# earth-insights/ZoomEarth

Hardware: AMD Instinct MI355X
Metric: questions/sec end-to-end, ZoomEarth-3B on 5000px tiles (higher is better)
Workload: dtype bf16

## Files before the change

### include/zoomearth.h

```cpp
#ifndef ZOOMEARTH_H
#define ZOOMEARTH_H

#include <stddef.h>
#include <stdint.h>

#ifdef __cplusplus
extern "C" {
#endif

typedef struct ze_engine ze_engine;

typedef enum {
    ZE_OK = 0,
    ZE_ERR_INVALID = -1,
    ZE_ERR_HIP = -2,
    ZE_ERR_NOMEM = -3,
    ZE_ERR_NOTFOUND = -4,
    ZE_ERR_MISMATCH = -5
} ze_status;

typedef enum { ZE_F32 = 0, ZE_F16 = 1, ZE_BF16 = 2 } ze_dtype;

#define ZE_MAX_FULLATT 16
#define ZE_MAX_EOS 4
// ... 170 lines not shown
                      float* out_rows, int32_t* out_stop, void* stream);

#define ZE_MAX_GRAMMARS 16
#define ZE_MAX_GRAMMAR_STATES 2048
#define ZE_MAX_GRAMMAR_CLASSES 4096
int ze_grammar_create(ze_engine* e, const uint16_t* token_class, int n_classes, const int16_t* trans, int n_states,
                      const uint8_t* accepting, int* out_grammar, void* stream);
int ze_grammar_destroy(ze_engine* e, int grammar);
int ze_seq_set_grammar(ze_engine* e, int seq, int grammar, int state, void* stream);
int ze_chain_grammar_state(ze_engine* e, int seq, int* state, int* violated, void* stream);
int ze_op_grammar_mask(ze_engine* e, int grammar, const float* logits, int rows, int vocab, int ld, const int32_t* states, float* out,
                       void* stream);
int ze_op_grammar_advance(ze_engine* e, int grammar, const int32_t* states, const int32_t* tokens, int rows, int32_t* out_states,
                          void* stream);

int ze_weights_quantize_fp8(ze_engine* e, void* stream);
int ze_set_fp8_activations(ze_engine* e, int on);
int ze_op_quantize_fp8(ze_engine* e, void* w_bf16, int rows, int cols, void* q_out, void* scale_out, void* stream);
int ze_op_linear_mx(ze_engine* e, const void* a8, const void* sa, const void* w8, const void* sw, const void* bias, void* c,
                    int M, int N, int K, int swiglu, void* stream);

#define ZE_WEIGHTS_BF16 0
#define ZE_WEIGHTS_FP8 1
#define ZE_WEIGHTS_MXFP4 2
int ze_weights_quantize_mxfp4(ze_engine* e, void* stream);
int ze_op_quantize_mxfp4(ze_engine* e, void* w_bf16, int rows, int cols, void* q_out, void* scale_out, void* stream);
int ze_op_gemv4(ze_engine* e, int epi, const void* q4, const void* scale_e8m0, const void* x_bf16, const void* norm_w, float eps,
                const void* bias_bf16, int N, int K, void* out_bf16, float* out_f32, const uint8_t* seen, float penalty,
                int32_t* out_token, int seq, int layer, const void* embed, int token, void* embed_out, void* stream);
int ze_weight_format(ze_engine* e);

int ze_op_linear(ze_engine* e, const void* a_bf16, const void* w_bf16, const void* bias_bf16, void* c_bf16, int M,
                 int N, int K, int act, void* stream);
int ze_op_rmsnorm(ze_engine* e, const void* x_bf16, const void* weight_bf16, void* y_bf16, int rows, int cols,
                  float eps, void* stream);
int ze_op_token_logprob(ze_engine* e, const void* logits_bf16, int rows, int vocab, int ld, const int32_t* targets,
                        float* out, void* stream);
int ze_op_score_detail(ze_engine* e, const void* logits_bf16, int rows, int vocab, int ld, const int32_t* targets, int top_n,
                       float* out_logprob, float* out_entropy, int32_t* out_rank, int32_t* out_top_ids, float* out_top_logprobs,
                       void* stream);
int ze_op_attention(ze_engine* e, const void* q, const void* k, const void* v, void* o, int T, int heads,
                    int kv_heads, int D, const int32_t* cu_seqlens, int n_seg, int causal, void* stream);

int ze_op_window_gather(ze_engine* e, const float* pixel_values, const int32_t* grid_thw, int n_images, void* out_bf16, void* stream);
int ze_op_window_scatter(ze_engine* e, const void* x_bf16, int cols, const int32_t* grid_thw, int n_images, void* out_bf16,
                         void* stream);
int ze_op_vision_rope(ze_engine* e, void* qkv_bf16, const int32_t* grid_thw, int n_images, int window_order, void* stream);
int ze_op_embed_scatter(ze_engine* e, const int32_t* input_ids, int len, const void* image_embeds, int n_image_rows, void* out_bf16,
                        void* stream);
int ze_op_mrope_kv(ze_engine* e, int seq, int layer, void* qkv_bf16, int T, const int32_t* position_ids, int past, void* stream);
int ze_op_rope_kv_decode(ze_engine* e, const int32_t* seqs, int n, int layer, void* qkv_bf16, void* stream);
int ze_op_kv_read(ze_engine* e, int seq, int layer, int start, int n, void* out_k, void* out_v, void* stream);

int ze_seq_set_speculation(ze_engine* e, int seq, int k, int min_ngram, int max_ngram, const int32_t* prompt_ids, int n_prompt, void* stream);
int ze_chain_spec_stats(ze_engine* e, int seq, int* steps, int* drafted, int* accepted, void* stream);
int ze_op_spec_draft(ze_engine* e, const int32_t* hist_ids, const int32_t* hist_lens, int rows, int ld, int k, int min_ngram,
                     int max_ngram, int32_t* out_draft, int32_t* out_len, void* stream);
int ze_op_spec_accept(ze_engine* e, const float* logits, int n_chains, int vocab, int ld, int k, const int32_t* draft,
                      const int32_t* draft_len, uint8_t* seen, const float* repetition_penalty, const int32_t* room, int ignore_eos,
                      int32_t* out_tokens, int32_t* out_count, int32_t* out_finished, void* stream);
int ze_op_decode_rows(ze_engine* e, int seq, const int32_t* tokens, int r, float* out_logits, void* stream);
int ze_op_attn_decode(ze_engine* e, const int32_t* seqs, int n, int layer, const void* qkv_bf16, void* out_bf16, void* stream);
int ze_op_attn_decode_single(ze_engine* e, int seq, int layer, const void* qkv_bf16, void* out_bf16, void* stream);
int ze_op_gemv(ze_engine* e, int epi, const void* w_bf16, const void* w8, const void* scale8, const void* x_bf16, const void* norm_w,
               float eps, const void* bias_bf16, int act8, int N, int K, void* out_bf16, float* out_f32, const uint8_t* seen,
               float penalty, int32_t* out_token, int seq, int layer, const void* embed, int token, void* embed_out, void* stream);
// ... 20 lines not shown
```

### zoomearth_amd/_lib.py

```python
from __future__ import annotations

import ctypes as C
import os
import subprocess

_HERE = os.path.dirname(os.path.abspath(__file__))
LIB_PATH = os.environ.get("ZE_LIB_PATH") or os.path.join(_HERE, "libzoomearth_hip.so")
CSRC = os.path.join(_HERE, "csrc")

ZE_F32, ZE_F16, ZE_BF16 = 0, 1, 2
ZE_MAX_FULLATT, ZE_MAX_EOS = 16, 4


class ZeConfig(C.Structure):
    _fields_ = [
        ("vit_depth", C.c_int32), ("vit_hidden", C.c_int32), ("vit_heads", C.c_int32),
        ("vit_intermediate", C.c_int32), ("vit_out_hidden", C.c_int32),
        ("patch_size", C.c_int32), ("temporal_patch_size", C.c_int32), ("spatial_merge_size", C.c_int32),
        ("window_size", C.c_int32), ("in_channels", C.c_int32),
        ("n_fullatt", C.c_int32), ("fullatt_block_indexes", C.c_int32 * ZE_MAX_FULLATT),
        ("hidden", C.c_int32), ("layers", C.c_int32), ("heads", C.c_int32), ("kv_heads", C.c_int32),
        ("intermediate", C.c_int32), ("vocab", C.c_int32),
        ("rms_eps", C.c_float), ("rope_theta", C.c_float), ("mrope_section", C.c_int32 * 3),
        ("tie_word_embeddings", C.c_int32),
# ... 130 lines not shown
                                         C.POINTER(C.c_float), _P, _P]),
    "ze_op_sample_rows": (C.c_int, [_P, _P, C.c_int, C.c_int, C.c_int, _P, C.POINTER(C.c_float), C.POINTER(C.c_float),
                                    C.POINTER(C.c_uint64), C.POINTER(C.c_int32), C.POINTER(C.c_int32), C.POINTER(C.c_int32),
                                    C.POINTER(C.c_float), C.POINTER(C.c_float), _P, _P]),
    "ze_seq_set_logprobs": (C.c_int, [_P, C.c_int, C.c_int, _P]),
    "ze_chain_logprobs": (C.c_int, [_P, C.c_int, C.POINTER(C.c_float), C.POINTER(C.c_int32), C.POINTER(C.c_float), C.c_int,
                                    C.POINTER(C.c_int), C.POINTER(C.c_int), _P]),
    "ze_chain_logprobs_batch": (C.c_int, [_P, C.POINTER(C.c_int32), C.c_int, C.POINTER(C.c_float), C.POINTER(C.c_int32),
                                          C.POINTER(C.c_float), C.c_int, C.c_int, C.POINTER(C.c_int32), _P]),
    "ze_op_token_logprobs": (C.c_int, [_P, _P, C.c_int, C.c_int, C.c_int, _P, C.c_int, _P, _P, _P, _P]),
    "ze_seq_set_logit_adjust": (C.c_int, [_P, C.c_int, C.c_float, C.c_float, C.c_int, C.POINTER(C.c_int32), C.POINTER(C.c_float),
                                          C.c_int, _P]),
    "ze_op_logit_adjust": (C.c_int, [_P, _P, C.c_int, C.c_int, C.c_int, _P, _P, _P, _P, _P, _P, _P, _P, _P]),
    "ze_seq_set_token_rules": (C.c_int, [_P, C.c_int, C.c_int, C.POINTER(C.c_int32), C.c_int, C.POINTER(C.c_int32), C.c_int,
                                         C.POINTER(C.c_int32), C.c_int, _P]),
    "ze_op_token_rules": (C.c_int, [_P, _P, C.c_int, C.c_int, C.c_int, _P, _P, _P, _P, _P, _P, _P, _P, _P, _P, _P, _P]),
    "ze_grammar_create": (C.c_int, [_P, C.POINTER(C.c_uint16), C.c_int, C.POINTER(C.c_int16), C.c_int, C.POINTER(C.c_uint8),
                                    C.POINTER(C.c_int), _P]),
    "ze_grammar_destroy": (C.c_int, [_P, C.c_int]),
    "ze_seq_set_grammar": (C.c_int, [_P, C.c_int, C.c_int, C.c_int, _P]),
    "ze_chain_grammar_state": (C.c_int, [_P, C.c_int, C.POINTER(C.c_int), C.POINTER(C.c_int), _P]),
    "ze_op_grammar_mask": (C.c_int, [_P, C.c_int, _P, C.c_int, C.c_int, C.c_int, _P, _P, _P]),
    "ze_op_grammar_advance": (C.c_int, [_P, C.c_int, _P, _P, C.c_int, _P, _P]),
    "ze_weights_quantize_fp8": (C.c_int, [_P, _P]),
    "ze_set_fp8_activations": (C.c_int, [_P, C.c_int]),
    "ze_op_quantize_fp8": (C.c_int, [_P, _P, C.c_int, C.c_int, _P, _P, _P]),
    "ze_weights_quantize_mxfp4": (C.c_int, [_P, _P]),
    "ze_op_quantize_mxfp4": (C.c_int, [_P, _P, C.c_int, C.c_int, _P, _P, _P]),
    "ze_op_gemv4": (C.c_int, [_P, C.c_int, _P, _P, _P, _P, C.c_float, _P, C.c_int, C.c_int, _P, _P, _P, C.c_float,
                              C.POINTER(C.c_int32), C.c_int, C.c_int, _P, C.c_int, _P, _P]),
    "ze_weight_format": (C.c_int, [_P]),
    "ze_op_linear_mx": (C.c_int, [_P, _P, _P, _P, _P, _P, _P, C.c_int, C.c_int, C.c_int, C.c_int, _P]),
    "ze_op_linear": (C.c_int, [_P, _P, _P, _P, _P, C.c_int, C.c_int, C.c_int, C.c_int, _P]),
    "ze_op_rmsnorm": (C.c_int, [_P, _P, _P, _P, C.c_int, C.c_int, C.c_float, _P]),
    "ze_op_attention": (C.c_int, [_P, _P, _P, _P, _P, C.c_int, C.c_int, C.c_int, C.c_int, C.POINTER(C.c_int32),
                                  C.c_int, C.c_int, _P]),
    "ze_op_window_gather": (C.c_int, [_P, _P, C.POINTER(C.c_int32), C.c_int, _P, _P]),
    "ze_op_window_scatter": (C.c_int, [_P, _P, C.c_int, C.POINTER(C.c_int32), C.c_int, _P, _P]),
    "ze_op_vision_rope": (C.c_int, [_P, _P, C.POINTER(C.c_int32), C.c_int, C.c_int, _P]),
    "ze_op_embed_scatter": (C.c_int, [_P, C.POINTER(C.c_int32), C.c_int, _P, C.c_int, _P, _P]),
    "ze_op_mrope_kv": (C.c_int, [_P, C.c_int, C.c_int, _P, C.c_int, C.POINTER(C.c_int32), C.c_int, _P]),
    "ze_op_rope_kv_decode": (C.c_int, [_P, C.POINTER(C.c_int32), C.c_int, C.c_int, _P, _P]),
    "ze_op_attn_decode": (C.c_int, [_P, C.POINTER(C.c_int32), C.c_int, C.c_int, _P, _P, _P]),
    "ze_op_attn_decode_single": (C.c_int, [_P, C.c_int, C.c_int, _P, _P, _P]),
    "ze_op_kv_read": (C.c_int, [_P, C.c_int, C.c_int, C.c_int, C.c_int, _P, _P, _P]),
    "ze_seq_set_speculation": (C.c_int, [_P, C.c_int, C.c_int, C.c_int, C.c_int, C.POINTER(C.c_int32), C.c_int, _P]),
    "ze_chain_spec_stats": (C.c_int, [_P, C.c_int, C.POINTER(C.c_int), C.POINTER(C.c_int), C.POINTER(C.c_int), _P]),
    "ze_op_spec_draft": (C.c_int, [_P, _P, _P, C.c_int, C.c_int, C.c_int, C.c_int, C.c_int, _P, _P, _P]),
    "ze_op_spec_accept": (C.c_int, [_P, _P, C.c_int, C.c_int, C.c_int, C.c_int, _P, _P, _P, _P, _P, C.c_int, _P, _P, _P, _P]),
    "ze_op_decode_rows": (C.c_int, [_P, C.c_int, C.POINTER(C.c_int32), C.c_int, _P, _P]),
    "ze_op_gemv": (C.c_int, [_P, C.c_int, _P, _P, _P, _P, _P, C.c_float, _P, C.c_int, C.c_int, C.c_int, _P, _P, _P, C.c_float,
                             C.POINTER(C.c_int32), C.c_int, C.c_int, _P, C.c_int, _P, _P]),
    "ze_op_logits_rows": (C.c_int, [_P, _P, _P, C.c_float, _P, _P, C.c_int, C.c_int, C.c_int, _P]),
    "ze_op_numeric_helpers": (C.c_int, [_P, _P, _P, _P, _P, C.c_int, _P]),
    "ze_profile_decode_kernel": (C.c_int, [_P, C.c_int, C.c_int, C.POINTER(C.c_float), C.POINTER(C.c_double), _P]),
    "ze_profile_batch_kernel": (C.c_int, [_P, C.c_int, C.c_int, C.c_int, C.POINTER(C.c_float), C.POINTER(C.c_double), _P]),
    "ze_profile_prefill_kernel": (C.c_int, [_P, C.c_int, C.c_int, C.c_int, C.POINTER(C.c_float), C.POINTER(C.c_double), _P]),
    "ze_profile_prefill_layer": (C.c_int, [_P, C.c_int, C.c_int, C.POINTER(C.c_float), C.POINTER(C.c_double), _P]),
    "ze_phase_timers": (C.c_int, [_P, C.c_int, C.c_int, C.POINTER(C.c_float)]),
    "ze_tune": (C.c_int, [C.c_int, C.c_int]),
}
EXPORTS = tuple(_SIGS)


def lib():
    global _lib
# ... 25 lines not shown
```

### zoomearth_amd/csrc/ze_forward.hip

```cpp
#include <math.h>
#include <cmath>
#include <string.h>

#include <algorithm>

#include "ze_engine.h"

extern int ze_gemv_knobs[24];

static int frontend_acquire(ze_engine* e) {
    if (e->fe_in_flight) {
        ZE_HIP(hipEventSynchronize(e->fe_done));
        e->fe_in_flight = false;
    }
    return ZE_OK;
}
static int frontend_release(ze_engine* e, hipStream_t s) {
    if (!e->fe_done) ZE_HIP(hipEventCreateWithFlags(&e->fe_done, hipEventDisableTiming));
    ZE_HIP(hipEventRecord(e->fe_done, s));
    e->fe_in_flight = true;
    return ZE_OK;
}
static int stage_acquire(ze_engine* e, hipEvent_t& ev) {
    if (ev) ZE_HIP(hipEventSynchronize(ev));
// ... 2122 lines not shown
        if (act == 5)
            ze_launch_gemm_oneshot(ZE_EPI_NONE, xf, wf, (const bf16_t*)bias, nullptr, 0, (bf16_t*)cmat, N, M, N, K, s);
        else
            ze_launch_gemm_frag(ZE_EPI_NONE, xf, wf, (const bf16_t*)bias, nullptr, 0, (bf16_t*)cmat, N, M, N, K, s);
        hipStreamSynchronize(s);
        hipFree(wf);
    } else if (act == 4) {
        if (N % 32) return ze_fail(e, ZE_ERR_INVALID, "SwiGLU: N = 2 * width with width % 16 == 0");
        ze_launch_gemm(ZE_EPI_SWIGLU, (const bf16_t*)a, K, (const bf16_t*)w, K, (const bf16_t*)bias, nullptr, 0,
                       (bf16_t*)cmat, N / 2, nullptr, M, N, K, s, e->prefill_ws());
    } else if (act == 6 || act == 7) {
        if (act == 7 && N % 32) return ze_fail(e, ZE_ERR_INVALID, "SwiGLU: N = 2 * width with width % 16 == 0");
        ze_launch_gemm_wide(act == 7 ? ZE_EPI_SWIGLU : ZE_EPI_NONE, (const bf16_t*)a, K, (const bf16_t*)w, K, (const bf16_t*)bias,
                            nullptr, 0, (bf16_t*)cmat, act == 7 ? N / 2 : N, M, N, K, e->gemm_ws(), s);
    } else if (act == 10) {
        ze_launch_gemm_wide(ZE_EPI_F32, (const bf16_t*)a, K, (const bf16_t*)w, K, nullptr, nullptr, 0, (bf16_t*)cmat, N, M, N, K,
                            e->gemm_ws(), s);
    } else if (act == 8 || act == 9) {
        if (act == 9 && N % 32) return ze_fail(e, ZE_ERR_INVALID, "SwiGLU: N = 2 * width with width % 16 == 0");
        if (K % 64 || K < 64) return ze_fail(e, ZE_ERR_INVALID, "eight-phase kernel: K a multiple of 64");
        ze_launch_gemm_p8(act == 9 ? ZE_EPI_SWIGLU : ZE_EPI_NONE, (const bf16_t*)a, K, (const bf16_t*)w, K, (const bf16_t*)bias, nullptr, 0,
                          (bf16_t*)cmat, act == 9 ? N / 2 : N, nullptr, M, N, K, s, e->prefill_ws());
    } else if (act == 2) {
        ze_launch_gemm_stream(ZE_EPI_NONE, (const bf16_t*)a, K, (const bf16_t*)w, K, (const bf16_t*)bias, nullptr, 0,
                              (bf16_t*)cmat, N, M, N, K, e->gemm_ws(), s);
    } else {
        ze_launch_gemm(act ? ZE_EPI_GELU : ZE_EPI_NONE, (const bf16_t*)a, K, (const bf16_t*)w, K, (const bf16_t*)bias,
                       nullptr, 0, (bf16_t*)cmat, N, nullptr, M, N, K, s, e->prefill_ws());
    }
    ZE_KCHECK();
    return ZE_OK;
}

extern "C" int ze_op_token_logprob(ze_engine* e, const void* logits, int rows, int vocab, int ld, const int32_t* targets,
                                   float* out, void* stream) {
    if (!logits || !targets || !out || rows < 0 || vocab <= 0 || ld < vocab || ld % 8)
        return ze_fail(e, ZE_ERR_INVALID, "bad token_logprob arguments");
    hipSetDevice(e->device);
    ze_launch_token_logprob((const bf16_t*)logits, ld, vocab, targets, out, rows, (hipStream_t)stream);
    ZE_KCHECK();
    return ZE_OK;
}

extern "C" int ze_op_score_detail(ze_engine* e, const void* logits, int rows, int vocab, int ld, const int32_t* targets, int top_n,
                                  float* out_logprob, float* out_entropy, int32_t* out_rank, int32_t* out_top_ids,
                                  float* out_top_logprobs, void* stream) {
    if (!e || !logits || !targets || !out_logprob || rows < 0 || vocab <= 0 || ld < vocab || ld % 8)
        return ze_fail(e, ZE_ERR_INVALID, "bad score_detail arguments");
    if (top_n < 0 || top_n > ZE_MAX_TOP_LOGPROBS) return ze_fail(e, ZE_ERR_INVALID, "top_n must be in [0, 20]");
    if (!out_top_ids != !out_top_logprobs || (out_top_ids && top_n < 1))
        return ze_fail(e, ZE_ERR_INVALID, "the top arrays are both null, or both set with top_n >= 1");
    hipSetDevice(e->device);
    ze_launch_score_detail((const bf16_t*)logits, ld, vocab, targets, out_top_ids ? top_n : 0, out_logprob, out_entropy, out_rank,
                           out_top_ids, out_top_logprobs, rows, (hipStream_t)stream);
    ZE_KCHECK();
    return ZE_OK;
}

extern "C" int ze_op_rmsnorm(ze_engine* e, const void* x, const void* weight, void* y, int rows, int cols, float eps,
                             void* stream) {
    if (!e || !x || !weight || !y) return ze_fail(e, ZE_ERR_INVALID, "null argument");
    if (cols % 8) return ze_fail(e, ZE_ERR_INVALID, "cols must be a multiple of 8");
    hipSetDevice(e->device);
    ze_launch_rmsnorm((const bf16_t*)x, cols, (const bf16_t*)weight, (bf16_t*)y, cols, rows, cols, eps,
                      (hipStream_t)stream);
    ZE_KCHECK();
// ... 508 lines not shown
```

### zoomearth_amd/csrc/ze_gemm.hip

```cpp
#include <algorithm>
#include <type_traits>

#include "ze_kernels.h"

typedef __attribute__((ext_vector_type(8))) __bf16 bf16x8;
typedef __attribute__((ext_vector_type(4))) float f32x4;
typedef __attribute__((ext_vector_type(4))) unsigned int u32x4;

#define GEMM_BK 64

extern int ze_live_engines;
extern int ze_gemv_knobs[24];

__device__ __forceinline__ float gelu_erf(float x) { return 0.5f * x * (1.0f + erff(x * 0.70710678118654752440f)); }

template <int BM, int BN, int EPI, int WM = 2, int WN = 2, bool LDS_EPI = false>
__device__ __forceinline__ void gemm_finish(f32x4 (&acc)[BM / (16 * WM)][BN / (16 * WN)], uint8_t* smem, const bf16_t* __restrict__ bias,
                                            const bf16_t* __restrict__ R, int ldr, bf16_t* __restrict__ C, int ldc,
                                            const int* __restrict__ c_rows, int M, int N, int ksplit, int ks, int bid,
                                            int nwg, int bm0, int bn0, float* __restrict__ slab,
                                            unsigned* __restrict__ tickets) {
    constexpr int TM = BM / (16 * WM), TN = BN / (16 * WN), NT = 64 * WM * WN;
    const int tid = threadIdx.x, lane = tid & 63, wid = tid >> 6;
    const int wm0 = (wid / WN) * (BM / WM), wn0 = (wid % WN) * (BN / WN);
// ... 643 lines not shown
            for (int i = 0; i < TM; ++i) {
#pragma unroll
                for (int j = 0; j < TN; ++j)
                    acc[i][j] = __builtin_amdgcn_mfma_f32_16x16x32_bf16(fa[i], fb[j], acc[i][j], 0, 0, 0);
                if (SPREAD && more) {
                    const int r = kk * TM + i;
#pragma unroll
                    for (int pc = 0; pc < LPW; ++pc)
                        if ((STAGES == 2 ? min(pc, 2 * TM - 1) : pc * (2 * TM) / LPW) == r) {
                            if (pc < LPA)
                                ring_issue_one(A, lda, bm0, M - 1, k_next, img_next, wid + pc * (NT / 64), lane);
                            else
                                ring_issue_one(W, ldw, bn0, N - 1, k_next, img_next + BM * 128,
                                               wid + (pc - LPA) * (NT / 64), lane);
                        }
                }
            }
        }
    }
    __syncthreads();
    gemm_finish<BM, BN, EPI, WM, WN, WIDE_EPI>(acc, smem, bias, R, ldr, C, ldc, c_rows, M, N, ksplit, ks, bid, nwg, bm0, bn0, slab, tickets);
}


template <int EPI>
__device__ __forceinline__ void p8_finish_wide(f32x4 (&acc)[8][4], uint8_t* scratch, const bf16_t* __restrict__ bias,
                                               const bf16_t* __restrict__ R, int ldr, bf16_t* __restrict__ C, int ldc,
                                               const int* __restrict__ c_rows, int M, int N, int row_base, int col_base, int lane) {
    constexpr bool SW = EPI == ZE_EPI_SWIGLU, F32 = EPI == ZE_EPI_F32;
    constexpr int EB = F32 ? 4 : 2;
    constexpr int OW = SW ? 32 : 64;
    constexpr int ROWB = OW * EB;
    constexpr int PPR = ROWB / 16;
    constexpr int CR = 4096 / ROWB > 32 ? 32 : 4096 / ROWB;
    constexpr int TI = CR / 16;
    const int fr = lane & 15, fq = lane >> 4;
    float b[4];
#pragma unroll
    for (int j = 0; j < 4; ++j) {
        const int ncol = col_base + j * 16 + fr;
        b[j] = (bias && ncol < N) ? bf16_to_f32(bias[ncol]) : 0.f;
    }
    const int ocol_base = SW ? col_base / 2 : col_base, on = SW ? N / 2 : N;
#pragma unroll
    for (int c = 0; c < 128 / CR; ++c) {
#pragma unroll
        for (int ii = 0; ii < TI; ++ii) {
            const int i = TI * c + ii;
#pragma unroll
            for (int j = 0; j < 4; j += (SW ? 2 : 1)) {
#pragma unroll
                for (int r = 0; r < 4; ++r) {
                    const int lrow = ii * 16 + fq * 4 + r;
                    const int swz = (lrow & (PPR - 1)) << 4;
                    float v;
                    int col;
                    if (SW) {
                        const float g = bf16_round(acc[i][j][r] + b[j]);
                        const float u = bf16_round(acc[i][j + 1][r] + b[j + 1]);
                        v = bf16_round(silu_f(g)) * u;
                        col = (j / 2) * 16 + fr;
                    } else {
                        v = bf16_round(acc[i][j][r] + b[j]);
                        if (EPI == ZE_EPI_GELU) v = gelu_erf(v);
                        col = j * 16 + fr;
                    }
                    if (F32) *reinterpret_cast<float*>(scratch + lrow * ROWB + ((col * 4) ^ swz)) = v;
                    else *reinterpret_cast<bf16_t*>(scratch + lrow * ROWB + ((col * 2) ^ swz)) = f32_to_bf16(v);
                }
            }
        }
        asm volatile("s_waitcnt lgkmcnt(0)" ::: "memory");
        constexpr int RPI = 64 / PPR;
#pragma unroll
        for (int it = 0; it < CR / RPI; ++it) {
            const int lrow = it * RPI + lane / PPR, piece = lane % PPR;
            uint4 v = *reinterpret_cast<const uint4*>(scratch + lrow * ROWB + ((piece ^ (lrow & (PPR - 1))) << 4));
            const int row = row_base + c * CR + lrow;
            const int col = ocol_base + piece * (16 / EB);
            if (row < M && col < on) {
                const int orow = c_rows ? c_rows[row] : row;
                if (EPI == ZE_EPI_RESIDUAL) {
                    const uint4 rr = *reinterpret_cast<const uint4*>(R + (size_t)row * ldr + col);
                    const uint32_t* pv = reinterpret_cast<const uint32_t*>(&v);
                    const uint32_t* pr = reinterpret_cast<const uint32_t*>(&rr);
                    uint32_t o[4];
#pragma unroll
                    for (int q = 0; q < 4; ++q) {
                        const float lo = __uint_as_float(pr[q] << 16) + __uint_as_float(pv[q] << 16);
                        const float hi = __uint_as_float(pr[q] & 0xffff0000u) + __uint_as_float(pv[q] & 0xffff0000u);
                        o[q] = (uint32_t)f32_to_bf16(lo) | ((uint32_t)f32_to_bf16(hi) << 16);
                    }
                    v = make_uint4(o[0], o[1], o[2], o[3]);
                }
                if (F32) *reinterpret_cast<uint4*>(reinterpret_cast<float*>(C) + (size_t)orow * ldc + col) = v;
                else *reinterpret_cast<uint4*>(C + (size_t)orow * ldc + col) = v;
            }
        }
        asm volatile("s_waitcnt lgkmcnt(0)" ::: "memory");
    }
}

__device__ __forceinline__ bool p8_splitk_reduce(f32x4 (&acc)[8][4], unsigned* flag, int ksplit, int ks, int bid, int nwg,
                                                 float* __restrict__ slab, unsigned* __restrict__ tickets) {
    constexpr int NT = 512, T = 32;
    const int tid = threadIdx.x;
    const size_t slab_bytes = (size_t)ksplit * nwg * NT * T * 16;
    auto rsrc = __builtin_amdgcn_make_buffer_rsrc(slab, 0, (int)min(slab_bytes, (size_t)0x7fffffff), 0x00020000);
    {
        const unsigned base = (unsigned)(((size_t)(ks * nwg + bid) * T * NT + tid) * 16);
#pragma unroll
        for (int i = 0; i < 8; ++i)
#pragma unroll
            for (int j = 0; j < 4; ++j) {
                u32x4 v;
                v.x = __float_as_uint(acc[i][j][0]);
                v.y = __float_as_uint(acc[i][j][1]);
                v.z = __float_as_uint(acc[i][j][2]);
                v.w = __float_as_uint(acc[i][j][3]);
                __builtin_amdgcn_raw_buffer_store_b128(v, rsrc, base + (unsigned)(i * 4 + j) * NT * 16, 0, 16 );
            }
    }
    asm volatile("s_waitcnt vmcnt(0)" ::: "memory");
    __syncthreads();
    if (tid == 0) {
// ... 61 lines not shown
            const int per_full = nmaj * CB, full = nmin / CB;
            int panel, o, cw;
            if (bid < full * per_full) { panel = bid / per_full; o = bid % per_full; cw = CB; }
            else { panel = full; o = bid - full * per_full; cw = nmin - full * CB; }
            const int per_rb = RB * cw, fb = nmaj / RB;
            int rb, oo, rw;
            if (o < fb * per_rb) { rb = o / per_rb; oo = o % per_rb; rw = RB; }
            else { rb = fb; oo = o - fb * per_rb; rw = nmaj - fb * RB; }
            const int tmaj = rb * RB + oo % rw, tmin = panel * CB + oo / rw;
            bm0 = (col_major ? tmaj : tmin) * BM;
            bn0 = (col_major ? tmin : tmaj) * BN;
            return;
        }
        bm0 = (col_major ? bid % nby : bid / nbx) * BM;
        bn0 = (col_major ? bid / nby : bid % nbx) * BN;
    };
    unsigned offA[2][2], offB[2][2];
    auto sources = [&]() {
#pragma unroll
        for (int h = 0; h < 2; ++h)
#pragma unroll
            for (int q = 0; q < 2; ++q) {
                const int hr = (wid * 2 + q) * 8 + (lane >> 3);
                const int c = (lane & 7) ^ ((hr >> 1) & 7);
                const int ra = min(bm0 + (hr >> 6) * 128 + h * 64 + (hr & 63), M - 1);
                const int rb = min(bn0 + (hr >> 5) * 64 + h * 32 + (hr & 31), N - 1);
                offA[h][q] = (unsigned)(((size_t)ra * lda + c * 8) * sizeof(bf16_t));
                offB[h][q] = (unsigned)(((size_t)rb * ldw + c * 8) * sizeof(bf16_t));
            }
    };
    auto stage = [&](int slot, int t) {
        const unsigned dst = smem_lds + (t & 1) * BUF + slot * HALF + wid * 2048;
        const bf16_t* base = (slot < 2 ? A : W) + (size_t)(kt0 + t) * GEMM_BK;
#pragma unroll
        for (int q = 0; q < 2; ++q) {
            const unsigned off = slot == 0 ? offA[0][q] : slot == 1 ? offA[1][q] : slot == 2 ? offB[0][q] : offB[1][q];
            unsigned keep;
            asm volatile("s_mov_b32 %0, m0\n\ts_mov_b32 m0, %2\n\ts_nop 0\n\tglobal_load_lds_dwordx4 %1, %3\n\ts_mov_b32 m0, %0"
                         : "=&s"(keep)
                         : "v"(off), "s"(dst + q * 1024), "s"(base)
                         : "memory");
        }
    };
    auto prologue = [&]() {
        stage(0, 0);
        stage(2, 0);
        stage(3, 0);
        stage(1, 0);
        if (nk > 1) {
            stage(0, 1);
            stage(2, 1);
            stage(3, 1);
        }
    };
    const int sw = (fr >> 1) & 7;
    const unsigned aoff0 = (wr * 64 + fr) * 128 + (((0 + fq) ^ sw) << 4), aoff1 = (wr * 64 + fr) * 128 + (((4 + fq) ^ sw) << 4);
    const unsigned boff0 = (wc * 32 + fr) * 128 + (((0 + fq) ^ sw) << 4), boff1 = (wc * 32 + fr) * 128 + (((4 + fq) ^ sw) << 4);
    bf16x8 fa[2][4], fb0[2][2], fb1[2][2];
    f32x4 acc[8][4];
    auto read_a = [&](int b, int mh) {
        const uint8_t* p = smem + b * BUF + mh * HALF;
#pragma unroll
        for (int i = 0; i < 4; ++i) {
            fa[0][i] = *reinterpret_cast<const bf16x8*>(p + aoff0 + i * 2048);
            fa[1][i] = *reinterpret_cast<const bf16x8*>(p + aoff1 + i * 2048);
        }
    };
    auto read_b = [&](bf16x8 (&f)[2][2], int b, int nh) {
        const uint8_t* p = smem + b * BUF + (2 + nh) * HALF;
#pragma unroll
        for (int j = 0; j < 2; ++j) {
            f[0][j] = *reinterpret_cast<const bf16x8*>(p + boff0 + j * 2048);
            f[1][j] = *reinterpret_cast<const bf16x8*>(p + boff1 + j * 2048);
        }
    };
    auto quadrant = [&](int mh, int nh, const bf16x8 (&f)[2][2]) {
        __builtin_amdgcn_s_setprio(1);
#pragma unroll
        for (int kk = 0; kk < 2; ++kk)
#pragma unroll
            for (int i = 0; i < 4; ++i)
#pragma unroll
                for (int j = 0; j < 2; ++j)
                    acc[mh * 4 + i][nh * 2 + j] = __builtin_amdgcn_mfma_f32_16x16x32_bf16(fa[kk][i], f[kk][j], acc[mh * 4 + i][nh * 2 + j], 0, 0, 0);
        __builtin_amdgcn_s_setprio(0);
    };

    const int nunits = nwg * ksplit;
    int tile = blockIdx.x;
    if (tile >= nunits) return;
    place(tile);
    sources();
    prologue();
    for (;;) {
#pragma unroll
        for (int i = 0; i < 8; ++i)
#pragma unroll
            for (int j = 0; j < 4; ++j) acc[i][j] = f32x4{0.f, 0.f, 0.f, 0.f};
        if (tile == (int)blockIdx.x && nk > 1) ring_wait<6>();
        else ring_wait<0>();
        __builtin_amdgcn_s_barrier();
        if (wr == 1) __builtin_amdgcn_s_barrier();

        for (int t = 0; t < nk; ++t) {
            const int b = t & 1;
            read_a(b, 0);
            __builtin_amdgcn_sched_barrier(0);
            read_b(fb0, b, 0);
            if (t + 1 < nk) stage(1, t + 1);
            asm volatile("s_waitcnt lgkmcnt(4)" ::: "memory");
            __builtin_amdgcn_s_barrier();
            quadrant(0, 0, fb0);
            __builtin_amdgcn_s_barrier();
            read_b(fb1, b, 1);
            if (t + 2 < nk) stage(0, t + 2);
            __builtin_amdgcn_s_barrier();
            quadrant(0, 1, fb1);
// ... 23 lines not shown
            prologue();
        }
        bool finish = true;
        if (ksplit > 1)
            finish = p8_splitk_reduce(acc, reinterpret_cast<unsigned*>(smem + 2 * BUF), ksplit, done_ks, done_bid, nwg, slab, tickets);
        if (!finish) {
            if (!more) break;
            continue;
        }
        if constexpr (WIDE)
            p8_finish_wide<EPI>(acc, smem + 2 * BUF + wid * 4096, bias, R, ldr, C, ldc, c_rows, M, N, done_bm0 + wr * 128, done_bn0 + wc * 64, lane);
        else
            gemm_finish<BM, BN, EPI, 2, 4>(acc, smem, bias, R, ldr, C, ldc, c_rows, M, N, 1, 0, done_bid, nwg, done_bm0, done_bn0, nullptr, nullptr);
        if (!more) break;
    }
}

static void launch_p8(int epi, const bf16_t* A, int lda, const bf16_t* W, int ldw, const bf16_t* bias, const bf16_t* R, int ldr,
                      bf16_t* C, int ldc, const int* c_rows, int M, int N, int K, hipStream_t s, int ksplit = 1,
                      const ze_gemm_ws& ws = ze_gemm_ws()) {
    static int cus = 0;
    if (!cus) {
        int dev = 0;
        hipGetDevice(&dev);
        if (hipDeviceGetAttribute(&cus, hipDeviceAttributeMultiprocessorCount, dev) != hipSuccess || cus <= 0) cus = 256;
        cus = std::max(8, cus / 8 * 8);
    }
    const int tiles = ze_cdiv(M, 256) * ze_cdiv(N, 256);
    const bool shared_gpu = ze_gemv_knobs[4] == 1 || (ze_gemv_knobs[4] == 0 && ze_live_engines > 1);
    const int units = tiles * std::max(1, ksplit);
    const int grid = (ze_gemv_knobs[7] == 9 || shared_gpu) ? units : std::min(units, cus);
    const bool sw = epi == ZE_EPI_SWIGLU;
    const bool wide = ze_gemv_knobs[7] != 10 && (ldc % 8) == 0 && ((size_t)C % 16) == 0 && ((sw ? N / 2 : N) % 8) == 0 &&
                      (epi != ZE_EPI_RESIDUAL || ((ldr % 8) == 0 && ((size_t)R % 16) == 0));
    const size_t lds = wide ? (128 + 32) * 1024 : (128 + 1) * 1024;
    const int blk = ze_gemv_knobs[21] == 1 ? 0 : (ze_gemv_knobs[21] > 1 ? ze_gemv_knobs[21] : ((8 << 8) | 4));
#define ZE_P8_LAUNCH(E, WD)                                                                                                    \
    do {                                                                                                                       \
        static bool attr_set = false;                                                                                          \
        if (!attr_set) {                                                                                                       \
            hipFuncSetAttribute(reinterpret_cast<const void*>(&k_gemm_p8<E, WD>), hipFuncAttributeMaxDynamicSharedMemorySize, (int)lds); \
            attr_set = true;                                                                                                   \
        }                                                                                                                      \
        hipLaunchKernelGGL((k_gemm_p8<E, WD>), dim3(grid), dim3(512), lds, s, A, lda, W, ldw, bias, R, ldr, C, ldc, c_rows, M, N, K, blk, \
                           std::max(1, ksplit), ws.slab, ws.tickets);                                                          \
    } while (0)
    if (wide) {
        switch (epi) {
            case ZE_EPI_NONE: ZE_P8_LAUNCH(ZE_EPI_NONE, true); break;
            case ZE_EPI_GELU: ZE_P8_LAUNCH(ZE_EPI_GELU, true); break;
            case ZE_EPI_RESIDUAL: ZE_P8_LAUNCH(ZE_EPI_RESIDUAL, true); break;
            case ZE_EPI_SWIGLU: ZE_P8_LAUNCH(ZE_EPI_SWIGLU, true); break;
            case ZE_EPI_F32: ZE_P8_LAUNCH(ZE_EPI_F32, true); break;
        }
        return;
    }
    switch (epi) {
        case ZE_EPI_NONE: ZE_P8_LAUNCH(ZE_EPI_NONE, false); break;
        case ZE_EPI_GELU: ZE_P8_LAUNCH(ZE_EPI_GELU, false); break;
        case ZE_EPI_RESIDUAL: ZE_P8_LAUNCH(ZE_EPI_RESIDUAL, false); break;
        case ZE_EPI_SWIGLU: ZE_P8_LAUNCH(ZE_EPI_SWIGLU, false); break;
        case ZE_EPI_F32: ZE_P8_LAUNCH(ZE_EPI_F32, false); break;
    }
#undef ZE_P8_LAUNCH
}

template <int BM, int BN, int SA, int DW, int NK, int EPI>
// ... 1088 lines not shown
```

### zoomearth_amd/engine.py

```python
from __future__ import annotations

import ctypes as C
import os
from typing import Iterable, NamedTuple, Optional, Sequence

import numpy as np
import torch

from . import _lib
from .config import ModelConfig

MAX_TOP_LOGPROBS = 20
MAX_LOGIT_BIAS = 512
MAX_RULE_INTS, MAX_RULE_WORDS, MAX_RULE_LEN = 1024, 64, 16
MAX_GRAMMARS = 16


def pack_records(records) -> np.ndarray:
    out = []
    for r in records:
        r = [int(t) for t in r]
        out.append(len(r))
        out.extend(r)
    return np.asarray(out, dtype=np.int32)
# ... 1037 lines not shown
        f32 = epi == self.GV_LOGITS
        self._check(self.lib.ze_op_gemv4(self.h, epi, _ptr(q4), _ptr(scale4), _ptr(x), _ptr(norm_w), eps, _ptr(bias), n, k,
                                         None if f32 else _ptr(out), _ptr(out) if f32 else None, _ptr(seen), penalty,
                                         C.byref(tok) if argmax else None, seq, layer, _ptr(embed), int(token), _ptr(embed_out),
                                         self._stream()))
        return (out, int(tok.value)) if argmax else out

    def op_logits_rows(self, x: torch.Tensor, w: torch.Tensor, norm_w: torch.Tensor, eps: float = 1e-6, out=None) -> torch.Tensor:
        rows, k = x.shape
        n = w.shape[0]
        if out is None:
            out = torch.empty((rows, n), dtype=torch.float32, device=self.device)
        self._check(self.lib.ze_op_logits_rows(self.h, _ptr(w), _ptr(norm_w), eps, _ptr(x), _ptr(out), rows, n, k, self._stream()))
        return out

    def op_numeric_helpers(self, x: torch.Tensor, y: torch.Tensor):
        n = x.numel()
        out = torch.empty(n, dtype=torch.int32, device=self.device)
        out2 = torch.empty(n, dtype=torch.int32, device=self.device)
        self._check(self.lib.ze_op_numeric_helpers(self.h, _ptr(x), _ptr(y), _ptr(out), _ptr(out2), n, self._stream()))
        return out, out2

    def op_linear(self, a, w, bias=None, act: int = 0):
        m, k = a.shape
        n = w.shape[0]
        if act == 10:
            out = torch.empty((m, n), dtype=torch.float32, device=self.device)
            self._check(self.lib.ze_op_linear(self.h, _ptr(a), _ptr(w), None, _ptr(out), m, n, k, act, self._stream()))
            return out
        out = torch.empty((m, n // 2 if act in (4, 7, 9) else n), dtype=torch.bfloat16, device=self.device)
        self._check(self.lib.ze_op_linear(self.h, _ptr(a), _ptr(w), _ptr(bias), _ptr(out), m, n, k, act, self._stream()))
        return out

    def op_rmsnorm(self, x, w, eps: float):
        out = torch.empty_like(x)
        self._check(self.lib.ze_op_rmsnorm(self.h, _ptr(x), _ptr(w), _ptr(out), x.shape[0], x.shape[1], eps,
                                           self._stream()))
        return out

    def op_attention(self, q, k, v, cu_seqlens, causal: bool):
        t, heads, d = q.shape
        kvh = k.shape[1]
        out = torch.empty_like(q)
        cu, cp = _i32(cu_seqlens)
        self._check(self.lib.ze_op_attention(self.h, _ptr(q), _ptr(k), _ptr(v), _ptr(out), t, heads, kvh, d, cp,
                                             len(cu) - 1, int(causal), self._stream()))
        return out

    def profile_decode_kernel(self, which: int, iters: int = 72):
        us, by = C.c_float(), C.c_double()
        self._check(self.lib.ze_profile_decode_kernel(self.h, which, iters, C.byref(us), C.byref(by), self._stream()))
        return float(us.value), float(by.value)

    def profile_batch_kernel(self, which: int, n: int, iters: int = 72):
        us, by = C.c_float(), C.c_double()
        self._check(self.lib.ze_profile_batch_kernel(self.h, which, n, iters, C.byref(us), C.byref(by), self._stream()))
        return float(us.value), float(by.value)

    def profile_prefill_kernel(self, which: int, rows: int, iters: int = 12):
        us, fl = C.c_float(), C.c_double()
        self._check(self.lib.ze_profile_prefill_kernel(self.h, which, rows, iters, C.byref(us), C.byref(fl), self._stream()))
        return float(us.value), float(fl.value)

    def profile_prefill_layer(self, rows: int, layers_run: int = 36):
        us, fl = (C.c_float * 4)(), (C.c_double * 4)()
        self._check(self.lib.ze_profile_prefill_layer(self.h, rows, layers_run, us, fl, self._stream()))
# ... 7 lines not shown
```

Before: 71.51.

## Transpose MFMA operands in wide p8 GEMM epilogue for packed vector LDS writes

In the wide eight-phase GEMM path, the MFMA operands are swapped so each lane holds four consecutive output columns. The epilogue can then pack bf16 pairs and write 8- or 16-byte chunks to LDS with a new swizzle, instead of scalar per-element stores. The bias is loaded as uint2 vectors, and the two global_load_lds issues are merged into one asm block. It also adds a bias-alignment condition for the wide path and a test entry point for the p8 GEMM. The new swizzle, half-swap fixups and larger chunk rows are intricate and risk layout bugs.

```diff
diff --git a/include/zoomearth.h b/include/zoomearth.h
--- a/include/zoomearth.h
+++ b/include/zoomearth.h
@@ -226,6 +226,8 @@
 
 int ze_op_linear(ze_engine* e, const void* a_bf16, const void* w_bf16, const void* bias_bf16, void* c_bf16, int M,
                  int N, int K, int act, void* stream);
+int ze_op_linear_p8(ze_engine* e, const void* a_bf16, const void* w_bf16, const void* bias_bf16, const void* r_bf16, int ldr,
+                    void* c, int ldc, const int32_t* c_rows, int M, int N, int K, int epi, void* stream);
 int ze_op_rmsnorm(ze_engine* e, const void* x_bf16, const void* weight_bf16, void* y_bf16, int rows, int cols,
                   float eps, void* stream);
 int ze_op_token_logprob(ze_engine* e, const void* logits_bf16, int rows, int vocab, int ld, const int32_t* targets,
diff --git a/zoomearth_amd/_lib.py b/zoomearth_amd/_lib.py
--- a/zoomearth_amd/_lib.py
+++ b/zoomearth_amd/_lib.py
@@ -186,6 +186,7 @@
     "ze_weight_format": (C.c_int, [_P]),
     "ze_op_linear_mx": (C.c_int, [_P, _P, _P, _P, _P, _P, _P, C.c_int, C.c_int, C.c_int, C.c_int, _P]),
     "ze_op_linear": (C.c_int, [_P, _P, _P, _P, _P, C.c_int, C.c_int, C.c_int, C.c_int, _P]),
+    "ze_op_linear_p8": (C.c_int, [_P, _P, _P, _P, _P, C.c_int, _P, C.c_int, _P, C.c_int, C.c_int, C.c_int, C.c_int, _P]),
     "ze_op_rmsnorm": (C.c_int, [_P, _P, _P, _P, C.c_int, C.c_int, C.c_float, _P]),
     "ze_op_attention": (C.c_int, [_P, _P, _P, _P, _P, C.c_int, C.c_int, C.c_int, C.c_int, C.POINTER(C.c_int32),
                                   C.c_int, C.c_int, _P]),
diff --git a/zoomearth_amd/csrc/ze_forward.hip b/zoomearth_amd/csrc/ze_forward.hip
--- a/zoomearth_amd/csrc/ze_forward.hip
+++ b/zoomearth_amd/csrc/ze_forward.hip
@@ -2178,6 +2178,22 @@
     return ZE_OK;
 }
 
+extern "C" int ze_op_linear_p8(ze_engine* e, const void* a, const void* w, const void* bias, const void* r, int ldr, void* cmat, int ldc,
+                               const int32_t* c_rows, int M, int N, int K, int epi, void* stream) {
+    if (!e || !a || !w || !cmat) return ze_fail(e, ZE_ERR_INVALID, "null argument");
+    if (epi != ZE_EPI_NONE && epi != ZE_EPI_GELU && epi != ZE_EPI_RESIDUAL && epi != ZE_EPI_SWIGLU && epi != ZE_EPI_F32)
+        return ze_fail(e, ZE_ERR_INVALID, "eight-phase kernel: epilogue NONE, GELU, RESIDUAL, SWIGLU or F32");
+    if (M <= 0 || N <= 0 || K % 64 || K < 64) return ze_fail(e, ZE_ERR_INVALID, "eight-phase kernel: K a multiple of 64");
+    if (epi == ZE_EPI_SWIGLU && N % 32) return ze_fail(e, ZE_ERR_INVALID, "SwiGLU: N = 2 * width with width % 16 == 0");
+    if (ldc < (epi == ZE_EPI_SWIGLU ? N / 2 : N)) return ze_fail(e, ZE_ERR_INVALID, "ldc shorter than an output row");
+    if (epi == ZE_EPI_RESIDUAL && (!r || ldr < N)) return ze_fail(e, ZE_ERR_INVALID, "RESIDUAL: r with ldr >= N");
+    hipSetDevice(e->device);
+    ze_launch_gemm_p8(epi, (const bf16_t*)a, K, (const bf16_t*)w, K, (const bf16_t*)bias, (const bf16_t*)r, ldr, (bf16_t*)cmat, ldc,
+                      c_rows, M, N, K, (hipStream_t)stream, e->prefill_ws());
+    ZE_KCHECK();
+    return ZE_OK;
+}
+
 extern "C" int ze_op_token_logprob(ze_engine* e, const void* logits, int rows, int vocab, int ld, const int32_t* targets,
                                    float* out, void* stream) {
     if (!logits || !targets || !out || rows < 0 || vocab <= 0 || ld < vocab || ld % 8)
diff --git a/zoomearth_amd/csrc/ze_gemm.hip b/zoomearth_amd/csrc/ze_gemm.hip
--- a/zoomearth_amd/csrc/ze_gemm.hip
+++ b/zoomearth_amd/csrc/ze_gemm.hip
@@ -699,15 +699,22 @@
     constexpr int OW = SW ? 32 : 64;
     constexpr int ROWB = OW * EB;
     constexpr int PPR = ROWB / 16;
-    constexpr int CR = 4096 / ROWB > 32 ? 32 : 4096 / ROWB;
+    constexpr int CR = 4096 / ROWB;
     constexpr int TI = CR / 16;
     const int fr = lane & 15, fq = lane >> 4;
-    float b[4];
+    float b[4][4];
 #pragma unroll
     for (int j = 0; j < 4; ++j) {
-        const int ncol = col_base + j * 16 + fr;
-        b[j] = (bias && ncol < N) ? bf16_to_f32(bias[ncol]) : 0.f;
-    }
+        const int ncol = col_base + j * 16 + fq * 4;
+        uint2 w = make_uint2(0u, 0u);
+        if (bias && ncol < N) w = *reinterpret_cast<const uint2*>(bias + ncol);
+        b[j][0] = bf16lo(w.x);
+        b[j][1] = bf16hi(w.x);
+        b[j][2] = bf16lo(w.y);
+        b[j][3] = bf16hi(w.y);
+    }
+    const int wswz = F32 ? (fq ^ fr) : (fq ^ (SW ? (fr >> 1) : (((fr & 7) << 1) | (fr >> 3))));
+    uint8_t* const wbase = scratch + fr * ROWB;
     const int ocol_base = SW ? col_base / 2 : col_base, on = SW ? N / 2 : N;
 #pragma unroll
     for (int c = 0; c < 128 / CR; ++c) {
@@ -715,25 +722,30 @@
         for (int ii = 0; ii < TI; ++ii) {
             const int i = TI * c + ii;
 #pragma unroll
-            for (int j = 0; j < 4; j += (SW ? 2 : 1)) {
-#pragma unroll
-                for (int r = 0; r < 4; ++r) {
-                    const int lrow = ii * 16 + fq * 4 + r;
-                    const int swz = (lrow & (PPR - 1)) << 4;
-                    float v;
-                    int col;
-                    if (SW) {
-                        const float g = bf16_round(acc[i][j][r] + b[j]);
-                        const float u = bf16_round(acc[i][j + 1][r] + b[j + 1]);
-                        v = bf16_round(silu_f(g)) * u;
-                        col = (j / 2) * 16 + fr;
+            for (int jo = 0; jo < OW / 16; ++jo) {
+                uint8_t* const dst = wbase + ii * 16 * ROWB + (((jo * 4) ^ wswz) << (F32 ? 4 : 3));
+                if constexpr (SW) {
+                    const int j = 2 * jo;
+                    const uint32_t g01 = pack_bf16x2(acc[i][j][0] + b[j][0], acc[i][j][1] + b[j][1]);
+                    const uint32_t g23 = pack_bf16x2(acc[i][j][2] + b[j][2], acc[i][j][3] + b[j][3]);
+                    const uint32_t u01 = pack_bf16x2(acc[i][j + 1][0] + b[j + 1][0], acc[i][j + 1][1] + b[j + 1][1]);
+                    const uint32_t u23 = pack_bf16x2(acc[i][j + 1][2] + b[j + 1][2], acc[i][j + 1][3] + b[j + 1][3]);
+                    const uint32_t s01 = pack_bf16x2(silu_f(bf16lo(g01)), silu_f(bf16hi(g01)));
+                    const uint32_t s23 = pack_bf16x2(silu_f(bf16lo(g23)), silu_f(bf16hi(g23)));
+                    *reinterpret_cast<uint2*>(dst) = make_uint2(pack_bf16x2(bf16lo(s01) * bf16lo(u01), bf16hi(s01) * bf16hi(u01)),
+                                                                pack_bf16x2(bf16lo(s23) * bf16lo(u23), bf16hi(s23) * bf16hi(u23)));
+                } else {
+                    const int j = jo;
+                    const uint32_t v01 = pack_bf16x2(acc[i][j][0] + b[j][0], acc[i][j][1] + b[j][1]);
+                    const uint32_t v23 = pack_bf16x2(acc[i][j][2] + b[j][2], acc[i][j][3] + b[j][3]);
+                    if constexpr (F32) {
+                        *reinterpret_cast<float4*>(dst) = make_float4(bf16lo(v01), bf16hi(v01), bf16lo(v23), bf16hi(v23));
+                    } else if constexpr (EPI == ZE_EPI_GELU) {
+                        *reinterpret_cast<uint2*>(dst) = make_uint2(pack_bf16x2(gelu_erf(bf16lo(v01)), gelu_erf(bf16hi(v01))),
+                                                                    pack_bf16x2(gelu_erf(bf16lo(v23)), gelu_erf(bf16hi(v23))));
                     } else {
-                        v = bf16_round(acc[i][j][r] + b[j]);
-                        if (EPI == ZE_EPI_GELU) v = gelu_erf(v);
-                        col = j * 16 + fr;
+                        *reinterpret_cast<uint2*>(dst) = make_uint2(v01, v23);
                     }
-                    if (F32) *reinterpret_cast<float*>(scratch + lrow * ROWB + ((col * 4) ^ swz)) = v;
-                    else *reinterpret_cast<bf16_t*>(scratch + lrow * ROWB + ((col * 2) ^ swz)) = f32_to_bf16(v);
                 }
             }
         }
@@ -742,7 +754,13 @@
 #pragma unroll
         for (int it = 0; it < CR / RPI; ++it) {
             const int lrow = it * RPI + lane / PPR, piece = lane % PPR;
-            uint4 v = *reinterpret_cast<const uint4*>(scratch + lrow * ROWB + ((piece ^ (lrow & (PPR - 1))) << 4));
+            const int pswz = F32 ? (lrow & 15) : SW ? ((lrow >> 2) & 3) : (lrow & 7);
+            uint4 v = *reinterpret_cast<const uint4*>(scratch + lrow * ROWB + ((piece ^ pswz) << 4));
+            if constexpr (SW) {
+                if ((lrow >> 1) & 1) v = make_uint4(v.z, v.w, v.x, v.y);
+            } else if constexpr (!F32) {
+                if (it & 1) v = make_uint4(v.z, v.w, v.x, v.y);
+            }
             const int row = row_base + c * CR + lrow;
             const int col = ocol_base + piece * (16 / EB);
             if (row < M && col < on) {
@@ -753,11 +771,8 @@
                     const uint32_t* pr = reinterpret_cast<const uint32_t*>(&rr);
                     uint32_t o[4];
 #pragma unroll
-                    for (int q = 0; q < 4; ++q) {
-                        const float lo = __uint_as_float(pr[q] << 16) + __uint_as_float(pv[q] << 16);
-                        const float hi = __uint_as_float(pr[q] & 0xffff0000u) + __uint_as_float(pv[q] & 0xffff0000u);
-                        o[q] = (uint32_t)f32_to_bf16(lo) | ((uint32_t)f32_to_bf16(hi) << 16);
-                    }
+                    for (int q = 0; q < 4; ++q)
+                        o[q] = pack_bf16x2(bf16lo(pr[q]) + bf16lo(pv[q]), bf16hi(pr[q]) + bf16hi(pv[q]));
                     v = make_uint4(o[0], o[1], o[2], o[3]);
                 }
                 if (F32) *reinterpret_cast<uint4*>(reinterpret_cast<float*>(C) + (size_t)orow * ldc + col) = v;
@@ -885,15 +900,14 @@
     auto stage = [&](int slot, int t) {
         const unsigned dst = smem_lds + (t & 1) * BUF + slot * HALF + wid * 2048;
         const bf16_t* base = (slot < 2 ? A : W) + (size_t)(kt0 + t) * GEMM_BK;
-#pragma unroll
-        for (int q = 0; q < 2; ++q) {
-            const unsigned off = slot == 0 ? offA[0][q] : slot == 1 ? offA[1][q] : slot == 2 ? offB[0][q] : offB[1][q];
-            unsigned keep;
-            asm volatile("s_mov_b32 %0, m0\n\ts_mov_b32 m0, %2\n\ts_nop 0\n\tglobal_load_lds_dwordx4 %1, %3\n\ts_mov_b32 m0, %0"
-                         : "=&s"(keep)
-                         : "v"(off), "s"(dst + q * 1024), "s"(base)
-                         : "memory");
-        }
+        const unsigned off0 = slot == 0 ? offA[0][0] : slot == 1 ? offA[1][0] : slot == 2 ? offB[0][0] : offB[1][0];
+        const unsigned off1 = slot == 0 ? offA[0][1] : slot == 1 ? offA[1][1] : slot == 2 ? offB[0][1] : offB[1][1];
+        unsigned keep;
+        asm volatile("s_mov_b32 %0, m0\n\ts_mov_b32 m0, %3\n\ts_nop 0\n\tglobal_load_lds_dwordx4 %1, %5\n\t"
+                     "s_mov_b32 m0, %4\n\ts_nop 0\n\tglobal_load_lds_dwordx4 %2, %5\n\ts_mov_b32 m0, %0"
+                     : "=&s"(keep)
+                     : "v"(off0), "v"(off1), "s"(dst), "s"(dst + 1024), "s"(base)
+                     : "memory");
     };
     auto prologue = [&]() {
         stage(0, 0);
@@ -935,7 +949,10 @@
             for (int i = 0; i < 4; ++i)
 #pragma unroll
                 for (int j = 0; j < 2; ++j)
-                    acc[mh * 4 + i][nh * 2 + j] = __builtin_amdgcn_mfma_f32_16x16x32_bf16(fa[kk][i], f[kk][j], acc[mh * 4 + i][nh * 2 + j], 0, 0, 0);
+                    if constexpr (WIDE)
+                        acc[mh * 4 + i][nh * 2 + j] = __builtin_amdgcn_mfma_f32_16x16x32_bf16(f[kk][j], fa[kk][i], acc[mh * 4 + i][nh * 2 + j], 0, 0, 0);
+                    else
+                        acc[mh * 4 + i][nh * 2 + j] = __builtin_amdgcn_mfma_f32_16x16x32_bf16(fa[kk][i], f[kk][j], acc[mh * 4 + i][nh * 2 + j], 0, 0, 0);
         __builtin_amdgcn_s_setprio(0);
     };
 
@@ -1025,7 +1042,8 @@
     const int grid = (ze_gemv_knobs[7] == 9 || shared_gpu) ? units : std::min(units, cus);
     const bool sw = epi == ZE_EPI_SWIGLU;
     const bool wide = ze_gemv_knobs[7] != 10 && (ldc % 8) == 0 && ((size_t)C % 16) == 0 && ((sw ? N / 2 : N) % 8) == 0 &&
-                      (epi != ZE_EPI_RESIDUAL || ((ldr % 8) == 0 && ((size_t)R % 16) == 0));
+                      (epi != ZE_EPI_RESIDUAL || ((ldr % 8) == 0 && ((size_t)R % 16) == 0)) &&
+                      ((size_t)bias % 8) == 0;
     const size_t lds = wide ? (128 + 32) * 1024 : (128 + 1) * 1024;
     const int blk = ze_gemv_knobs[21] == 1 ? 0 : (ze_gemv_knobs[21] > 1 ? ze_gemv_knobs[21] : ((8 << 8) | 4));
 #define ZE_P8_LAUNCH(E, WD)                                                                                                    \
diff --git a/zoomearth_amd/engine.py b/zoomearth_amd/engine.py
--- a/zoomearth_amd/engine.py
+++ b/zoomearth_amd/engine.py
@@ -1093,6 +1093,15 @@
         self._check(self.lib.ze_op_linear(self.h, _ptr(a), _ptr(w), _ptr(bias), _ptr(out), m, n, k, act, self._stream()))
         return out
 
+    def op_linear_p8(self, a, w, bias=None, epi: int = 0, residual=None, out=None, c_rows=None):
+        m, k = a.shape
+        n = w.shape[0]
+        if out is None:
+            out = torch.empty((m, n // 2 if epi == 3 else n), dtype=torch.float32 if epi == 4 else torch.bfloat16, device=self.device)
+        self._check(self.lib.ze_op_linear_p8(self.h, _ptr(a), _ptr(w), _ptr(bias), _ptr(residual), residual.stride(0) if residual is not None else 0,
+                                             _ptr(out), out.stride(0), _ptr(c_rows), m, n, k, epi, self._stream()))
+        return out
+
     def op_rmsnorm(self, x, w, eps: float):
         out = torch.empty_like(x)
         self._check(self.lib.ze_op_rmsnorm(self.h, _ptr(x), _ptr(w), _ptr(out), x.shape[0], x.shape[1], eps,
```

Result: slower. 70.21 (-1.8%).
